# wesselb/stheno

Measured on AMD Instinct MI355X. Metric: GP logpdf+posterior evals/sec at N=16384 D=8 fp64, higher is better.
Workload: dtype f64; 1 GPU; EQ() kernel, N=16384 D=8 fp64, logpdf + condition, posterior mean/var at N*=2048; nan_scan=every step (the library's per-tensor memo is cleared at the start of each step), call_order=posterior-first, info_check=behind the call that factorised (the library's default), parallelism=replicas only (1 independent evals in flight, one process per GPU)

## Files before the change

### stheno_amd/csrc/gpk_common.hpp

```cpp
#pragma once
#include <hip/hip_runtime.h>
#include <stdint.h>
#include "../../include/gpk.h"

#ifdef GPK_DEV_KNOBS
#define GPK_KNOB(type, name, value) type name = (value)
#define GPK_KNOB_SET(stmt) stmt
#else
#define GPK_KNOB(type, name, value) constexpr type name = (value)
#define GPK_KNOB_SET(stmt) ((void)0)
#endif

#define GPK_WAVE 64
#define GPK_TILE 128
#define GPK_DB 128

#define GPK_ERR_ARG(i) (-(i))

typedef double f64x4 __attribute__((ext_vector_type(4)));
typedef float f32x4 __attribute__((ext_vector_type(4)));
typedef double f64x2 __attribute__((ext_vector_type(2)));

template <typename T>
struct Traits;

template <>
struct Traits<double> {
    typedef f64x4 acc_t;
    typedef f64x2 vec_t;
    static constexpr int VEC = 2;
    static constexpr int BK = 16;
    static __device__ __forceinline__ acc_t mfma(double a, double b, acc_t c) {
        return __builtin_amdgcn_mfma_f64_16x16x4f64(a, b, c, 0, 0, 0);
    }
    static __device__ __forceinline__ int crow(int lane, int i) { return (lane >> 4) + 4 * i; }
    static __host__ __device__ constexpr int rowq(int j) { return j & 3; }
    static __host__ __device__ constexpr int rowi(int j) { return j >> 2; }
};

template <>
struct Traits<float> {
    typedef f32x4 acc_t;
    typedef f32x4 vec_t;
    static constexpr int VEC = 4;
    static constexpr int BK = 32;
    static __device__ __forceinline__ acc_t mfma(float a, float b, acc_t c) {
        return __builtin_amdgcn_mfma_f32_16x16x4f32(a, b, c, 0, 0, 0);
    }
    static __device__ __forceinline__ int crow(int lane, int i) { return (lane >> 4) * 4 + i; }
    static __host__ __device__ constexpr int rowq(int j) { return j >> 2; }
    static __host__ __device__ constexpr int rowi(int j) { return j & 3; }
};

static inline int64_t gpk_cdiv(int64_t a, int64_t b) { return (a + b - 1) / b; }

#if defined(__HIPCC__)
__device__ __forceinline__ void gpk_barrier_stores_done() {
    asm volatile("s_waitcnt vmcnt(0)" ::: "memory");
    __syncthreads();
}
#endif

#define GPK_CHECK_LAUNCH()                                   \
    do {                                                     \
        hipError_t e__ = hipGetLastError();                  \
        if (e__ != hipSuccess) return GPK_ERR_LAUNCH;        \
    } while (0)


static inline bool gpk_valid_sb(int sb) { return sb >= 128 && sb <= 4096 && (sb & (sb - 1)) == 0; }

template <typename T>
int gpk_gemm_launch(bool a_kmaj, bool b_kmaj, int64_t M, int64_t N, int64_t K, T alpha,
                    const T* A, int64_t lda, int64_t sA, const T* B, int64_t ldb, int64_t sB,
                    T beta, T* C, int64_t ldc, int64_t sC, int64_t batch, int flags,
                    hipStream_t stream);

template <typename T>
int gpk_gemm_launch2(bool a_kmaj, bool b_kmaj, int64_t M, int64_t N, int64_t K, T alpha,
                     const T* A, int64_t lda, int64_t sA, int64_t sA2, const T* B, int64_t ldb,
                     int64_t sB, int64_t sB2, T beta, T* C, int64_t ldc, int64_t sC, int64_t sC2,
                     int64_t batch, int64_t batch2, int flags, hipStream_t stream,
                     const T* colscale = nullptr, T* colss = nullptr, int64_t ldss = 0);

#define GPK_PERSIST_CTRL_WORDS 64
int gpk_helper_stream(hipStream_t* aux, unsigned keys[8]);
int gpk_helper_side_stream(hipStream_t* side);
void gpk_helper_shutdown();
void gpk_potrf_shutdown();
template <typename T>
struct GpkSeg {
    int64_t M, N, K;
    const T* A; int64_t lda;
    const T* B; int64_t ldb;
    const T* Cin; int64_t ldcin;
    T* C; int64_t ldc;
    int lower_only;
    int signal;
    uint64_t colmask;
    int64_t grp;
};
#define GPK_PERSIST_MAX_SEG 4
struct GpkPersistSaved {
    alignas(16) char bytes[2048];
    int ts, edge, per_cu, valid;
    int signal_tiles;
};
template <typename T>
int gpk_gemm_persist_launch(const GpkSeg<T>* segs, int nseg, T alpha, unsigned* ctrl, int reserve,
                            hipStream_t stream, GpkPersistSaved* saved = nullptr, bool ctrl_zeroed = false);
template <typename T>
int gpk_gemm_persist_rejoin(const GpkPersistSaved* saved, hipStream_t helper_stream);

template <typename T>
int gpk_panel_step_launch(T* A, int64_t n, int64_t ld, int64_t c, const T* W, int64_t ke, unsigned* flags, hipStream_t stream);

template <typename T>
int gpk_potrf_launch(T* A, int64_t n, int64_t ld, int64_t batch, int64_t bstride, T* dinv,
                     int* info, int nbo, hipStream_t stream);

int64_t gpk_potrf_la_ws_elems_impl(int64_t n, int nb);
template <typename T>
int gpk_potrf_la_launch(T* A, int64_t n, int64_t ld, T* dinv128, T* dinv_big, int nb, T* ws, int* info,
                        hipStream_t stream, int sb = 0, int64_t rows = 0, int flags = 0);

template <typename T>
int gpk_potrf_rows_launch(T* A, int64_t n, int64_t rows, int64_t ld, T* dinv, int* info, hipStream_t stream);

void* gpk_prof_begin(int variant, double flops, hipStream_t stream);
void gpk_prof_end(void* slot, hipStream_t stream);

void gpk_tune_gemm(int key, int64_t value);
void gpk_tune_potrf(int key, int64_t value);
void gpk_tune_kmat(int key, int64_t value);
void gpk_tune_kdiff(int key, int64_t value);
void gpk_tune_solve(int key, int64_t value);
void gpk_set_diag_prof(long long* dev_buf);
void gpk_set_tile_prof(long long* dev_buf);
// ... 118 lines not shown
```

### stheno_amd/csrc/gpk_gemm.hip

```cpp
#include "gpk_common.hpp"
#include "gpk_gemm_tile.hpp"
#include <type_traits>
#include <cstring>
#include <mutex>
#include <vector>

namespace {

__device__ __forceinline__ void tri_decode(int s, int& I, int& J) {
    int i = (int)((sqrtf(8.f * (float)s + 1.f) - 1.f) * 0.5f);
    while ((i + 1) * (i + 2) / 2 <= s) ++i;
    while (i * (i + 1) / 2 > s) --i;
    I = i;
    J = s - i * (i + 1) / 2;
}

template <typename T>
__device__ __forceinline__ bool decode_tile(const GemmArgs<T>& p, int bid, int& ti, int& tj) {
    const bool tri = p.lower_only && p.tiles_m == p.tiles_n;
    if (tri) {
        tri_decode(bid, ti, tj);
        return ti < p.tiles_m;
    }
    if (p.tri_k_lo_b) {
// ... 232 lines not shown
    int variant;
    double flops;
    bool ended;
};
struct Prof {
    bool on = false;
    std::vector<ProfSlot> used, pool;
    ProfSlot* begin(int variant, double flops, hipStream_t stream) {
        ProfSlot s;
        if (!pool.empty()) {
            s = pool.back();
            pool.pop_back();
        } else {
            if (hipEventCreate(&s.a) != hipSuccess || hipEventCreate(&s.b) != hipSuccess) return nullptr;
        }
        s.variant = variant;
        s.flops = flops;
        s.ended = false;
        (void)hipEventRecord(s.a, stream);
        used.push_back(s);
        return &used.back();
    }
    void end(ProfSlot* s, hipStream_t stream) { (void)hipEventRecord(s->b, stream); s->ended = true; }
};
Prof g_prof;

GPK_KNOB(int64_t, g_small_tile_below, 512);
GPK_KNOB(int, g_trib, 1);
GPK_KNOB(int, g_xcd_batch, 1);
GPK_KNOB(int, g_trilo_pairs, 1);
GPK_KNOB(int, g_split_tail, 1);

}

namespace {
long long* g_tile_prof = nullptr;
int64_t g_tile_prof_only = -1;
int64_t g_tile_prof_count = 0;
GPK_KNOB(int64_t, g_persist_small_below, 512);
int g_cu_count[64] = {0};
int device_cus() {
    int dev = 0;
    if (hipGetDevice(&dev) != hipSuccess || dev < 0 || dev >= 64) return 256;
    if (g_cu_count[dev] == 0) {
        int n = 0;
        if (hipDeviceGetAttribute(&n, hipDeviceAttributeMultiprocessorCount, dev) != hipSuccess || n <= 0) n = 256;
        g_cu_count[dev] = n;
    }
    return g_cu_count[dev];
}
}

void gpk_set_tile_prof(long long* dev_buf) { g_tile_prof = dev_buf; }

void gpk_tune_gemm(int key, int64_t value) {
    if (key == 1) GPK_KNOB_SET(g_small_tile_below = value;);
    if (key == 8) GPK_KNOB_SET(g_persist_small_below = value;);
    if (key == 31) GPK_KNOB_SET(g_split_tail = (int)value;);
    if (key == 36) GPK_KNOB_SET(g_trib = (int)value;);
    if (key == 42) GPK_KNOB_SET(g_trilo_pairs = (int)value;);
    if (key == 45) GPK_KNOB_SET(g_xcd_batch = (int)value;);
    if (key == 20) { g_tile_prof_only = value; g_tile_prof_count = 0; }
}

void* gpk_prof_begin(int variant, double flops, hipStream_t stream) { return g_prof.on ? (void*)g_prof.begin(variant, flops, stream) : nullptr; }
void gpk_prof_end(void* slot, hipStream_t stream) {
    if (slot != nullptr) g_prof.end(static_cast<ProfSlot*>(slot), stream);
}

extern "C" int gpk_prof_start(void) {
    for (auto& s : g_prof.used) g_prof.pool.push_back(s);
    g_prof.used.clear();
    g_prof.on = true;
    return GPK_OK;
}

extern "C" int gpk_prof_stop(int variant, double* total_ms, int64_t* launches, double* useful_flops) {
    g_prof.on = false;
    double ms = 0, fl = 0;
    int64_t n = 0;
    for (auto& s : g_prof.used) {
        if (!s.ended) continue;
        if (hipEventSynchronize(s.b) != hipSuccess) return GPK_ERR_LAUNCH;
        if (variant >= 0 && s.variant != variant) continue;
        float t = 0;
        if (hipEventElapsedTime(&t, s.a, s.b) != hipSuccess) return GPK_ERR_LAUNCH;
        ms += t;
        fl += s.flops;
        ++n;
    }
    if (total_ms) *total_ms = ms;
    if (launches) *launches = n;
    if (useful_flops) *useful_flops = fl;
    return GPK_OK;
}

template <typename T>
int gpk_gemm_launch2(bool a_kmaj, bool b_kmaj, int64_t M, int64_t N, int64_t K, T alpha,
                     const T* A, int64_t lda, int64_t sA, int64_t sA2, const T* B, int64_t ldb,
                     int64_t sB, int64_t sB2, T beta, T* C, int64_t ldc, int64_t sC, int64_t sC2,
                     int64_t batch, int64_t batch2, int flags, hipStream_t stream, const T* colscale, T* colss, int64_t ldss) {
    const bool lower_only = (flags & 1) != 0;
    const bool fused_cols = colscale != nullptr || colss != nullptr;
    if (fused_cols && (batch != 1 || batch2 != 1 || lower_only || (const void*)A == (const void*)C || (const void*)B == (const void*)C))
        return GPK_ERR_ARG(17);
    if (M <= 0 || N <= 0 || batch <= 0 || batch2 <= 0) return GPK_OK;
// ... 519 lines not shown
```

### stheno_amd/csrc/gpk_gemm_tile.hpp

```cpp
#pragma once
#include "gpk_common.hpp"
#include <type_traits>

#ifndef GPK_GEMM_PIPE
#define GPK_GEMM_PIPE 2
#endif
#ifndef GPK_GEMM_PIPE64
#define GPK_GEMM_PIPE64 1
#endif
namespace {

constexpr int op_bytes(int ts) { return (ts + 16) * 128; }
constexpr int64_t GPK_PIPE_LD_MAX = (int64_t)1 << 21;
constexpr int64_t GPK_C_LD_MAX = (int64_t)1 << 25;

template <typename T>
struct GemmArgs {
    const T* A;
    const T* B;
    T* C;
    const T* Cin;
    int64_t lda, ldb, ldc, ldcin, sA, sB, sC;
    int64_t sA2, sB2, sC2;
    int M, N, K;
    T alpha, beta_over_alpha;
    int has_beta;
    int tiles_m, tiles_n;
    int lower_only;
    int vec_ok;
    int tri_k;
    int tri_k_lo;
    int tri_k_lo_b;
    int pair_cols;
    const T* colscale;
    T* colss;
    int64_t ldss;
    int xcd_batch;
    int xcd_tiles;
    unsigned long long colmask;
    int grp_tiles;
    int split_from;
};

__device__ __forceinline__ int gpk_claim_task(unsigned* ctr) { return (int)atomicAdd(ctr, 1u); }

template <typename T, int TS, bool KMAJ, bool EDGE, int NT = 256>
__device__ __forceinline__ void gload(typename Traits<T>::vec_t (&r)[TS * 8 / NT], const T* __restrict__ base,
                                      int64_t ld, int r0, int k0, int R, int K, int tid, bool fast) {
    typedef typename Traits<T>::vec_t vec_t;
    constexpr int VEC = Traits<T>::VEC;
    if (KMAJ) {
        const int c = tid & 7, rr0 = tid >> 3;
#pragma unroll
        for (int i = 0; i < TS * 8 / NT; ++i) {
            const int row = r0 + rr0 + (NT / 8) * i;
            const int k = k0 + c * VEC;
            const T* p = base + (int64_t)row * ld + k;
            if (!EDGE || fast) {
                r[i] = *reinterpret_cast<const vec_t*>(p);
            } else {
#pragma unroll
                for (int v = 0; v < VEC; ++v) r[i][v] = (row < R && k + v < K) ? p[v] : T(0);
            }
        }
    } else {
        constexpr int CPR = TS / VEC;
#pragma unroll
        for (int i = 0; i < TS * 8 / NT; ++i) {
            const int id = tid + NT * i;
            const int krow = id / CPR, cc = id % CPR;
            const int k = k0 + krow;
            const int row = r0 + cc * VEC;
            const T* p = base + (int64_t)k * ld + row;
            if (!EDGE || fast) {
                r[i] = *reinterpret_cast<const vec_t*>(p);
            } else {
#pragma unroll
                for (int v = 0; v < VEC; ++v) r[i][v] = (k < K && row + v < R) ? p[v] : T(0);
            }
        }
    }
}

template <typename T, int TS, bool KMAJ, int NT = 256>
__device__ __forceinline__ void sstore(char* lds, const typename Traits<T>::vec_t (&r)[TS * 8 / NT], int tid) {
    typedef typename Traits<T>::vec_t vec_t;
    constexpr int VEC = Traits<T>::VEC;
    if (KMAJ) {
        const int c = tid & 7, rr0 = tid >> 3;
#pragma unroll
        for (int i = 0; i < TS * 8 / NT; ++i) {
            const int rr = rr0 + (NT / 8) * i;
            const int off = rr * 128 + ((c ^ ((rr >> 1) & 7)) << 4);
            *reinterpret_cast<vec_t*>(lds + off) = r[i];
        }
    } else {
        constexpr int CPR = TS / VEC;
#pragma unroll
// ... 511 lines not shown
```

### stheno_amd/csrc/gpk_potrf.hip

```cpp
#include "gpk_common.hpp"
#include "gpk_gemm_tile.hpp"
#include "gpk_potrf_pipe.hpp"
#include <vector>

namespace {

constexpr int LDP = 130;

template <typename T>
struct DiagArgs {
    T* A;
    int64_t ld, bstride, off;
    int n;
    T* dinv;
    int64_t dinv_bstride;
    int* info;
    int info_base;
    long long* prof;
    int zero_next;
    T* rhs = nullptr;
    int64_t rhs_stride = 0;
};

#define PROF_MARK(i)                                                            \
// ... 449 lines not shown
    }
    int lane = lane_fixed;
    asm volatile("" : "+v"(lane));
    if (!vec_io) {
        for (int idx = tid; idx < GPK_DB * GPK_DB; idx += D3_THREADS) {
            const int r = idx >> 7, c = idx & 127;
            if (r < nv && c <= r) A[(int64_t)r * ld + c] = S[r * LDP + c];
        }
    }
    if (W == nullptr) {
        if (vec_io && wave == 4) store_l_columns<T>(S, A, ld, 7, lane);
        return;
    }
    if (prof) prof[10] = (long long)__builtin_readcyclecounter();

    inverse_last_rows<T>(S, rdiag, D16, W, wave, lane, lane & 15, lane >> 4);
    if (vec_io && wave == 7) store_l_columns<T>(S, A, ld, 7, lane);
    if (prof) prof[12] = (long long)__builtin_readcyclecounter();
    if (zero_next && tid < 256) {
        uint4* z = reinterpret_cast<uint4*>(W + (int64_t)GPK_DB * GPK_DB);
        z[tid] = make_uint4(0u, 0u, 0u, 0u);
    }
    if (prof) prof[13] = (long long)__builtin_readcyclecounter();
}


template <typename T, int WPE = 2>
__global__ __launch_bounds__(D3_THREADS, WPE) void potrf_diag3_kernel(DiagArgs<T> p) {
    __shared__ __attribute__((aligned(16))) T S[D3_LDS_ELEMS];
    const int64_t b = blockIdx.x;
    T* A = p.A + b * p.bstride + p.off * p.ld + p.off;
    const int rem = p.n - (int)p.off;
    T* W = p.dinv == nullptr ? nullptr : p.dinv + b * p.dinv_bstride + (p.off / GPK_DB) * (int64_t)(GPK_DB * GPK_DB);
    long long* prof = (p.prof != nullptr && blockIdx.x == 0 && threadIdx.x == 0) ? p.prof + (p.off / GPK_DB) * 32 : nullptr;
    diag3_block<T, true>(S, S + GPK_DB * LDP, A, p.ld, rem < GPK_DB ? rem : GPK_DB, W, p.info + b, (int)p.off + p.info_base, p.zero_next, prof);
    if (p.rhs != nullptr && W != nullptr) {
        gpk_barrier_stores_done();
        const int tid = threadIdx.x;
        const int nv = rem < GPK_DB ? rem : GPK_DB;
        T* yb = p.rhs + b * p.rhs_stride + p.off;
        if (tid < GPK_DB) S[tid] = tid < nv ? yb[tid] : T(0);
        __syncthreads();
        const int row = tid >> 2, q = tid & 3;
        const T* wr = W + (int64_t)row * GPK_DB + q * 32;
        T acc = T(0);
#pragma unroll 8
        for (int k = 0; k < 32; ++k) acc += wr[k] * S[q * 32 + k];
        acc += __shfl_xor(acc, 1, 64);
        acc += __shfl_xor(acc, 2, 64);
        if (q == 0 && row < nv) yb[row] = acc;
    }
}

constexpr unsigned PIPE_SPIN_LIMIT = 1u << 22;

template <typename T>
struct PipeArgs {
    T* A;
    int64_t ld;
    int m;
    int w;
    PipeShape sh;
    T* dinv;
    unsigned* ctrl;
    int* info;
    int info_off;
    int vec_ok;
    int ntasks, nseg;
    int segoff[GPK_PIPE_MAX_SEGS + 1];
    long long* prof;
    unsigned* wait_word;
    unsigned wait_value;
    GemmArgs<T> fill;
    int fill_tiles;
    int panel_wgs;
};

__device__ __forceinline__ bool pipe_poll(unsigned* w, bool mine, unsigned want, unsigned* abort_word) {
    unsigned it = 0;
    for (;;) {
        const bool ok = !mine || __hip_atomic_load(w, __ATOMIC_RELAXED, __HIP_MEMORY_SCOPE_AGENT) == want;
        if (__all(ok)) return true;
        __builtin_amdgcn_s_sleep(2);
        if ((++it & 255u) == 0) {
            if (__hip_atomic_load(abort_word, __ATOMIC_RELAXED, __HIP_MEMORY_SCOPE_AGENT) != 0u) return false;
            if (it > PIPE_SPIN_LIMIT) {
                __hip_atomic_store(abort_word, 1u, __ATOMIC_RELAXED, __HIP_MEMORY_SCOPE_AGENT);
                return false;
            }
        }
    }
}

__device__ __forceinline__ bool pipe_wait(unsigned* w0, unsigned* w1, unsigned* w2, unsigned* w3, unsigned v0, unsigned v1,
                                          unsigned v2, unsigned v3, int count, unsigned* abort_word, int* s_ctl) {
    const int tid = threadIdx.x;
    if (tid < 64) {
        unsigned* w = tid == 0 ? w0 : (tid == 1 ? w1 : (tid == 2 ? w2 : w3));
        const unsigned v = tid == 0 ? v0 : (tid == 1 ? v1 : (tid == 2 ? v2 : v3));
        const bool mine = tid < count;
        const bool ok = pipe_poll(mine ? w : w0, mine, v, abort_word);
        if (tid == 0) {
            s_ctl[1] = ok ? 1 : 0;
            __builtin_amdgcn_fence(__ATOMIC_ACQUIRE, "agent");
        }
    }
    __syncthreads();
    return s_ctl[1] != 0;
}

__device__ __forceinline__ void pipe_publish(unsigned* word, unsigned v, unsigned* counter = nullptr, unsigned full = 0u) {
    gpk_barrier_stores_done();
    if (threadIdx.x == 0) {
        __builtin_amdgcn_fence(__ATOMIC_RELEASE, "agent");
        asm volatile("s_waitcnt vmcnt(0)" ::: "memory");
        if (counter == nullptr) {
            __hip_atomic_store(word, v, __ATOMIC_RELAXED, __HIP_MEMORY_SCOPE_AGENT);
        } else {
            const unsigned before = __hip_atomic_fetch_add(counter, 1u, __ATOMIC_RELAXED, __HIP_MEMORY_SCOPE_AGENT);
            if (word != nullptr && before + 1u == full) __hip_atomic_store(word, v, __ATOMIC_RELAXED, __HIP_MEMORY_SCOPE_AGENT);
        }
    }
}

template <typename T>
__device__ __forceinline__ void pipe_chain(const PipeArgs<T>& p, T* __restrict__ S, int* s_ctl) {
    T* rdiag = S + GPK_DB * LDP;
    const int tid = threadIdx.x;
    const int npb = p.sh.npb, nd = p.sh.nd;
    unsigned* abort_word = p.ctrl + 1;
    unsigned* cnt = p.ctrl + GPK_PIPE_CTRL_HEAD + (int64_t)p.sh.R * npb;
    int64_t ld = p.ld;
    for (int j = 0; j < nd; ++j) {
        asm volatile("" : "+s"(ld));
        T* Ab = p.A + (int64_t)GPK_DB * j * ld + GPK_DB * j;
        const int rem = p.m - GPK_DB * j;
        T* W = p.dinv + (int64_t)j * (GPK_DB * GPK_DB);
        long long* prof = (p.prof != nullptr && tid == 0) ? p.prof + j * 32 : nullptr;
        if (prof) prof[14] = (long long)__builtin_readcyclecounter();
        if (j > 0) {
            unsigned* c = cnt + (int64_t)(2 * j) * npb + j;
            if (!pipe_wait(c, c, c, c, (unsigned)pipe_xupdates(pipe_fine_strips(p.sh, j - 1)), 0u, 0u, 0u, 1, abort_word, s_ctl)) break;
        } else if (p.wait_word != nullptr) {
            if (!pipe_wait(p.wait_word, p.wait_word, p.wait_word, p.wait_word, p.wait_value, 0u, 0u, 0u, 1, abort_word, s_ctl)) break;
        }
// ... 589 lines not shown
        bool done = false;
        if (owed > 0) {
            const T* P = A + k0 * ld + (k0 - owed);
            int st = gpk_gemm_launch<T>(true, true, rows - k0, k1 - k0, owed, T(-1), P, ld, bstride, P, ld, bstride, T(1), A + k0 * ld + k0, ld,
                                        bstride, batch, true, stream);
            if (st) return st;
            if (k1 < n && n - k0 > GPK_DB) {
                st = potrf_panel_pipe<T>(ctx, k0, nbo, &done, owed);
                if (st) return st;
            }
            if (!done && k1 < n) {
                const T* P2 = A + k1 * ld + (k0 - owed);
                st = gpk_gemm_launch<T>(true, true, rows - k1, n - k1, owed, T(-1), P2, ld, bstride, P2, ld, bstride, T(1), A + k1 * ld + k1, ld,
                                        bstride, batch, true, stream);
                if (st) return st;
            }
            owed = 0;
        }
        if (!done) {
            int pst = potrf_panel_any<T>(ctx, k0, nbo);
            if (pst) return pst;
        }
        if (k1 < n) {
            if (ride && n - k1 > GPK_DB) {
                owed = k1 - k0;
            } else {
                const T* P = A + k1 * ld + k0;
                int st = gpk_gemm_launch<T>(true, true, rows - k1, n - k1, k1 - k0, T(-1), P, ld, bstride, P, ld,
                                            bstride, T(1), A + k1 * ld + k1, ld, bstride, batch, true, stream);
                if (st) return st;
            }
        }
    }
    return GPK_OK;
}


#include <mutex>

namespace {

struct LaDevice {
    hipStream_t aux = nullptr;
    hipStream_t priv = nullptr;
    std::vector<hipEvent_t> events;
};
std::mutex g_la_mutex;
LaDevice g_la_dev[64];
GPK_KNOB(int64_t, g_la_min_rows, 2048);
GPK_KNOB(int64_t, g_la_tail_rows, 0);
GPK_KNOB(int, g_la_mode, 1);
GPK_KNOB(int64_t, g_la_fuse_diag_rows, 9216);
GPK_KNOB(int, g_la_fuse_diag_nb, 512);
GPK_KNOB(int, g_la_agg, 2);
GPK_KNOB(int64_t, g_la_agg_min_rows, 0);

LaDevice* la_device() {
    int dev = 0;
    if (hipGetDevice(&dev) != hipSuccess || dev < 0 || dev >= 64) return nullptr;
    LaDevice& d = g_la_dev[dev];
    if (d.aux == nullptr) {
        unsigned keys[8];
        if (gpk_helper_stream(&d.aux, keys) != GPK_OK) d.aux = nullptr;
    }
    return &d;
}

hipEvent_t la_event(LaDevice& d, size_t i) {
    while (d.events.size() <= i) {
        hipEvent_t e;
        if (hipEventCreateWithFlags(&e, hipEventDisableTiming) != hipSuccess) return nullptr;
        d.events.push_back(e);
    }
    return d.events[i];
}

template <typename T>
int la_chain(T* A, int64_t n, int64_t ld, T* dinv128, T* dinv_big, int nb, int sb, T* tmp, int* info, int64_t j,
             hipStream_t s, int max_wgs = 0, unsigned* wait_word = nullptr, unsigned wait_value = 0) {
    const int64_t k0 = j * nb;
    const int64_t w = (n - k0 < nb) ? n - k0 : nb;
    T* Ab = A + k0 * ld + k0;
    T* d128 = dinv128 + (k0 / GPK_DB) * (int64_t)(GPK_DB * GPK_DB);
    PanelCtx<T> sub{Ab, w, ld, 1, 0, d128, 0, info, s, (int)k0, max_wgs, wait_word, wait_value};
    int st = potrf_panel_any<T>(sub, 0, nb);
    if (st) return st;
    return gpk_trtri_merge_launch<T>(Ab, w, ld, 1, 0, d128, sb, dinv_big + (k0 / sb) * (int64_t)sb * sb, tmp, s);
}

}

void gpk_potrf_shutdown() {
    std::lock_guard<std::mutex> lock(g_la_mutex);
    int cur = 0;
    (void)hipGetDevice(&cur);
    for (int dev = 0; dev < 64; ++dev) {
        LaDevice& d = g_la_dev[dev];
        if (d.aux == nullptr && d.priv == nullptr && d.events.empty()) continue;
        (void)hipSetDevice(dev);
        if (d.priv != nullptr) {
            (void)hipStreamSynchronize(d.priv);
            (void)hipStreamDestroy(d.priv);
        }
        for (hipEvent_t e : d.events) (void)hipEventDestroy(e);
        d = LaDevice();
    }
    (void)hipSetDevice(cur);
}

void gpk_tune_potrf(int key, int64_t value) {
    if (key == 6) GPK_KNOB_SET(g_la_min_rows = value;);
    if (key == 7) GPK_KNOB_SET(g_la_mode = (int)value;);
    if (key == 9) GPK_KNOB_SET(g_la_tail_rows = value;);
    if (key == 32) GPK_KNOB_SET(g_fused_step = (int)value;);
    if (key == 37) GPK_KNOB_SET(g_pipe = (int)value;);
    if (key == 40) GPK_KNOB_SET(g_la_fuse_diag_rows = value;);
    if (key == 41) GPK_KNOB_SET(g_la_fuse_diag_nb = (int)value;);
    if (key == 47) GPK_KNOB_SET(g_la_agg = (int)value;);
    if (key == 48) GPK_KNOB_SET(g_la_agg_min_rows = value;);
    if (key == 52) GPK_KNOB_SET(g_plain_nbo = value;);
    if (key == 53) GPK_KNOB_SET(g_batch_mixed = (int)value;);
    if (key == 54) GPK_KNOB_SET(g_batch_mixed_min = value;);
    if (key == 55) GPK_KNOB_SET(g_batch_lag = (int)value;);
    if (key == 57) GPK_KNOB_SET(g_diag_two_per_cu = (int)value;);
    if (key == 38) GPK_KNOB_SET(g_pipe_fill = (int)value;);
    if (key == 39) GPK_KNOB_SET(g_pipe_panel_wgs = (int)value;);
}

#define GPK_LA_PAD 16
int64_t gpk_potrf_la_ws_elems_impl(int64_t n, int nb) {
    return (n > nb ? n : nb) * (int64_t)(nb + GPK_LA_PAD) + (int64_t)nb * nb / 4 + 16 + 128 + nb;
}

template <typename T>
static int potrf_la_body(LaDevice* dev, T* A, int64_t n, int64_t ld, T* dinv128, T* dinv_big, int nb, int sb, T* ws, int* info,
                         hipStream_t stream, int64_t rows, int flags);

template <typename T>
int gpk_potrf_la_launch(T* A, int64_t n, int64_t ld, T* dinv128, T* dinv_big, int nb, T* ws, int* info,
                        hipStream_t stream, int sb, int64_t rows, int flags) {
    if (n <= 0) return GPK_OK;
    if (rows < n) rows = n;
    if ((flags & GPK_ROWS_RHS) && rows < n + GPK_ROWS_RHS_STRIP) return GPK_ERR_ARG(2);
    if (rows > INT32_MAX) return GPK_ERR_ARG(2);
    if (rows > n && n % GPK_DB != 0) return GPK_ERR_ARG(2);
    if (rows > n && gpk_cdiv(n, nb) > 64) return GPK_ERR_ARG(2);
    if (ld < n) return GPK_ERR_ARG(3);
    if (nb < 256 || nb > 4096 || (nb & (nb - 1))) return GPK_ERR_ARG(6);
    if (sb <= 0) sb = nb;
    if (sb < 256 || sb > nb || (sb & (sb - 1))) return GPK_ERR_ARG(10);
    if (dinv128 == nullptr || dinv_big == nullptr || ws == nullptr || info == nullptr) return GPK_ERR_ARG(4);

    std::lock_guard<std::mutex> lock(g_la_mutex);
    LaDevice* dev = la_device();
    if (dev == nullptr) return GPK_ERR_LAUNCH;
    if (stream != nullptr) return potrf_la_body<T>(dev, A, n, ld, dinv128, dinv_big, nb, sb, ws, info, stream, rows, flags);

    if (dev->priv == nullptr && hipStreamCreateWithFlags(&dev->priv, hipStreamNonBlocking) != hipSuccess) {
        dev->priv = nullptr;
        return GPK_ERR_LAUNCH;
    }
    hipEvent_t e_in = la_event(*dev, 0), e_out = la_event(*dev, 1);
    if (e_in == nullptr || e_out == nullptr) return GPK_ERR_LAUNCH;
    if (hipEventRecord(e_in, nullptr) != hipSuccess || hipStreamWaitEvent(dev->priv, e_in, 0) != hipSuccess) return GPK_ERR_LAUNCH;
    const int st = potrf_la_body<T>(dev, A, n, ld, dinv128, dinv_big, nb, sb, ws, info, dev->priv, rows, flags);
    if (hipEventRecord(e_out, dev->priv) != hipSuccess || hipStreamWaitEvent(nullptr, e_out, 0) != hipSuccess) return st ? st : GPK_ERR_LAUNCH;
    return st;
}

template <typename T>
static int potrf_la_body(LaDevice* dev, T* A, int64_t n, int64_t ld, T* dinv128, T* dinv_big, int nb, int sb, T* ws, int* info,
                         hipStream_t stream, int64_t rows, int flags) {
    const bool rhs = (flags & GPK_ROWS_RHS) != 0;
    const int64_t Rall = rows;
    const int64_t R = rhs ? rows - GPK_ROWS_RHS_STRIP : rows;
    T* bvec = rhs ? A + R * ld : nullptr;
    unsigned* const ctrl_sets[2] = {reinterpret_cast<unsigned*>(ws), reinterpret_cast<unsigned*>(ws) + GPK_PERSIST_CTRL_WORDS};
    const int64_t ldt = nb + GPK_LA_PAD;
    T* Tp = ws + 128;
    T* tmp = Tp + (Rall > nb ? Rall : nb) * ldt;
    T* vtmp = tmp + (int64_t)nb * nb / 4 + 16;
    const int64_t nblk = gpk_cdiv(n, nb);
    const int64_t per = (int64_t)sb * sb;
    size_t ev = 2;

    auto finish_plain = [&](int64_t k) -> int {
        int s = potrf_plain<T>(A + k * ld + k, n - k, ld, 1, 0, dinv128 + (k / GPK_DB) * (int64_t)(GPK_DB * GPK_DB), info,
                               0, (int)k, stream, Rall - k);
        if (s) return s;
        if (flags & GPK_ROWS_NO_TAIL_INVERSES) return GPK_OK;
        return gpk_trtri_merge_launch<T>(A + k * ld + k, n - k, ld, 1, 0, dinv128 + (k / GPK_DB) * (int64_t)(GPK_DB * GPK_DB),
                                         sb, dinv_big + (k / sb) * per, Tp, stream);
    };
    int64_t tail_rows = g_la_tail_rows > 0 ? g_la_tail_rows : 6144;
    if (Rall > n && tail_rows < nb) tail_rows = nb;
    if (n <= tail_rows) return finish_plain(0);

    hipEvent_t e_side = nullptr;
    bool side_used = false;
    hipStream_t side = nullptr;
    if (rhs && g_la_mode == 1 && dev->aux != nullptr && gpk_helper_side_stream(&side) != GPK_OK) side = nullptr;
    auto rhs_panel = [&](int64_t j) -> int {
        if (!rhs) return GPK_OK;
        hipStream_t s = stream;
        if (side != nullptr) {
            hipEvent_t e = la_event(*dev, ev++);
            if (e == nullptr || hipEventRecord(e, stream) != hipSuccess || hipStreamWaitEvent(side, e, 0) != hipSuccess) return GPK_ERR_LAUNCH;
            side_used = true;
            s = side;
        }
        const int64_t k0 = j * nb;
        for (int64_t c = 0; c < nb; c += sb) {
            const int64_t r0 = k0 + c, r1 = r0 + sb;
            const int st1 = gpk_trsv_step_launch<T>(dinv_big + (r0 / sb) * per, sb, sb, A + r1 * ld + r0, ld, n - r1, bvec + r0, bvec + r1, vtmp, s);
            if (st1) return st1;
        }
        return GPK_OK;
    };
    auto rhs_join = [&]() -> int {
        if (!side_used) return GPK_OK;
        if (e_side == nullptr) e_side = la_event(*dev, ev++);
        if (e_side == nullptr || hipEventRecord(e_side, side) != hipSuccess || hipStreamWaitEvent(stream, e_side, 0) != hipSuccess) return GPK_ERR_LAUNCH;
        return GPK_OK;
    };
    auto steps = [&]() -> int {
        int st = la_chain<T>(A, n, ld, dinv128, dinv_big, nb, sb, tmp, info, 0, stream);
        if (st) return st;
        if (nblk > 1) {
            st = gpk_copy2d_launch<T>(A + (int64_t)nb * ld, ld, 0, Tp + (int64_t)nb * ldt, ldt, 0, R - nb, nb, 1, stream);
            if (st) return st;
        }
        const int agg = (g_la_agg > 1 && nblk <= 64) ? (int)g_la_agg : 1;
        std::vector<int> applied((size_t)nblk, 0);
        struct ColGroup { int from; uint64_t mask; };
        auto group_cols = [&](int64_t c_first, int64_t j, bool all, std::vector<ColGroup>& out) {
            out.clear();
            const bool wide = nblk - c_first > 64;
            for (int64_t c = c_first; c < nblk; ++c) {
                if (!all && (c - j) % agg != 0) continue;
                size_t g = 0;
                while (g < out.size() && out[g].from != applied[(size_t)c]) ++g;
                if (g == out.size()) out.push_back(ColGroup{applied[(size_t)c], 0});
                if (wide) out[g].mask = ~(uint64_t)0;
                else out[g].mask |= (uint64_t)1 << (c - c_first);
                applied[(size_t)c] = (int)(j + 1);
            }
        };
        auto col_segment = [&](const ColGroup& cg, int64_t c_first, int64_t k1) -> GpkSeg<T> {
            const int64_t kc = c_first * nb, ka = (int64_t)cg.from * nb;
            const T* P = A + kc * ld + ka;
            const uint64_t every = (nblk - c_first >= 64) ? ~(uint64_t)0 : (((uint64_t)1 << (nblk - c_first)) - 1);
            return GpkSeg<T>{R - kc, n - kc, k1 - ka, P, ld, P, ld, A + kc * ld + kc, ld, A + kc * ld + kc, ld, 1, 0,
                             (cg.mask == every && R == n) ? 0 : cg.mask, nb};
        };
        std::vector<ColGroup> groups;
        for (int64_t j = 0; j + 1 < nblk; ++j) {
            const int64_t k0 = j * nb, k1 = k0 + nb;
            const int64_t k2 = (k1 + nb < n) ? k1 + nb : n;
            unsigned* const ctrl_step = ctrl_sets[j & 1];
            unsigned* const ctrl = ctrl_sets[(j + 1) & 1];
            if (sb < nb) {
                for (int64_t i = 0; i * sb < nb && st == GPK_OK; ++i) {
                    const int64_t c = i * sb;
                    if (i > 0)
                        st = gpk_gemm_launch<T>(true, true, R - k1, sb, c, T(-1), A + k1 * ld + k0, ld, 0, A + (k0 + c) * ld + k0, ld, 0, T(1),
                                                Tp + k1 * ldt + c, ldt, 0, 1, 0, stream);
                    if (st == GPK_OK)
                        st = gpk_gemm_launch<T>(true, true, R - k1, sb, sb, T(1), Tp + k1 * ldt + c, ldt, 0, dinv_big + (k0 / sb + i) * per, sb, 0, T(0),
                                                A + k1 * ld + k0 + c, ld, 0, 1, 8, stream);
                }
            } else {
                st = gpk_gemm_launch<T>(true, true, R - k1, nb, nb, T(1), Tp + k1 * ldt, ldt, 0, dinv_big + j * per, nb, 0, T(0),
                                        A + k1 * ld + k0, ld, 0, 1, 8, stream);
            }
            if (st) return st;
            st = rhs_panel(j);
            if (st) return st;
            if (n - k1 <= tail_rows) {
                group_cols(j + 1, j, true, groups);
                for (size_t g0 = 0; g0 < groups.size(); g0 += GPK_PERSIST_MAX_SEG) {
                    GpkSeg<T> sg[GPK_PERSIST_MAX_SEG];
                    int ns = 0;
                    for (size_t g = g0; g < groups.size() && ns < GPK_PERSIST_MAX_SEG; ++g) sg[ns++] = col_segment(groups[g], j + 1, k1);
                    st = gpk_gemm_persist_launch<T>(sg, ns, T(-1), ctrl, 0, stream);
                    if (st) return st;
                }
                st = rhs_join();
                if (st) return st;
                return finish_plain(k1);
            }
            const int64_t ka1 = (int64_t)applied[(size_t)(j + 1)] * nb, kd1 = k1 - ka1;
            applied[(size_t)(j + 1)] = (int)(j + 1);
            const T* P1 = A + k1 * ld + ka1;
            const bool overlap = g_la_mode == 1 && dev->aux != nullptr && (n - k2) >= g_la_min_rows;
            const bool fuse_diag = overlap && nb <= g_la_fuse_diag_nb && g_la_fuse_diag_rows > 0 && (n - k2) >= g_la_fuse_diag_rows && g_pipe &&
                                   (k2 - k1) > GPK_DB;
            if (!fuse_diag) {
                st = gpk_gemm_launch<T>(true, true, k2 - k1, k2 - k1, kd1, T(-1), P1, ld, 0, P1, ld, 0, T(1),
                                        A + k1 * ld + k1, ld, 0, 1, 1, stream);
                if (st) return st;
            }
            if (k2 < n) group_cols(j + 2, j, agg == 1 || (n - k2) < g_la_agg_min_rows, groups);
            else groups.clear();
            {
                const size_t room = (size_t)(GPK_PERSIST_MAX_SEG - 1 - (fuse_diag ? 1 : 0));
                while (groups.size() > room) {
                    GpkSeg<T> sg = col_segment(groups.back(), j + 2, k1);
                    groups.pop_back();
                    st = gpk_gemm_persist_launch<T>(&sg, 1, T(-1), ctrl, 0, stream);
                    if (st) return st;
                }
            }
            hipEvent_t e_fork = nullptr, e_join = nullptr;
            if (overlap) {
                e_fork = la_event(*dev, ev++);
                e_join = la_event(*dev, ev++);
                if (e_fork == nullptr || e_join == nullptr) return GPK_ERR_LAUNCH;
                if (hipMemsetAsync(ctrl_step, 0, GPK_PERSIST_CTRL_WORDS * sizeof(unsigned), stream) != hipSuccess) return GPK_ERR_LAUNCH;
                if (hipEventRecord(e_fork, stream) != hipSuccess) return GPK_ERR_LAUNCH;
            } else {
                st = la_chain<T>(A, n, ld, dinv128, dinv_big, nb, sb, tmp, info, j + 1, stream);
                if (st) return st;
            }
            GpkPersistSaved saved;
            saved.valid = 0;
            auto forked = [&]() -> int {
                if (k2 < n) {
                    const T* P2 = A + k2 * ld + ka1;
                    GpkSeg<T> seg[GPK_PERSIST_MAX_SEG];
                    int ns = 0;
                    if (fuse_diag) seg[ns++] = GpkSeg<T>{k2 - k1, k2 - k1, kd1, P1, ld, P1, ld, A + k1 * ld + k1, ld, A + k1 * ld + k1, ld, 1, 1};
                    const GpkSeg<T> strip{R - k2, k2 - k1, kd1, P2, ld, P1, ld, A + k2 * ld + k1, ld, Tp + k2 * ldt, ldt, 0};
                    for (const ColGroup& cg : groups) seg[ns++] = col_segment(cg, j + 2, k1);
                    seg[ns++] = strip;
                    const int s2 = gpk_gemm_persist_launch<T>(seg, ns, T(-1), ctrl_step, overlap ? 1 : 0, stream, &saved, overlap);
                    if (s2) return s2;
                }
                if (overlap) {
                    if (hipStreamWaitEvent(dev->aux, e_fork, 0) != hipSuccess) return GPK_ERR_LAUNCH;
                    const int s2 = fuse_diag ? la_chain<T>(A, n, ld, dinv128, dinv_big, nb, sb, tmp, info, j + 1, dev->aux, 8, ctrl_step + 2, (unsigned)saved.signal_tiles)
                                             : la_chain<T>(A, n, ld, dinv128, dinv_big, nb, sb, tmp, info, j + 1, dev->aux, 8);
                    if (s2) return s2;
                    if (saved.valid)
                        return gpk_gemm_persist_rejoin<T>(&saved, dev->aux);
                }
                return GPK_OK;
            };
            st = forked();
            if (overlap) {
                const bool joined = hipEventRecord(e_join, dev->aux) == hipSuccess && hipStreamWaitEvent(stream, e_join, 0) == hipSuccess;
                if (!joined && st == GPK_OK) st = GPK_ERR_LAUNCH;
            }
            if (st) return st;
        }
        return GPK_OK;
    };
    const int st_all = steps();
    const int st_join = rhs_join();
    return st_all ? st_all : st_join;
}

template int gpk_potrf_la_launch<double>(double*, int64_t, int64_t, double*, double*, int, double*, int*, hipStream_t, int, int64_t, int);
template int gpk_potrf_la_launch<float>(float*, int64_t, int64_t, float*, float*, int, float*, int*, hipStream_t, int, int64_t, int);

template <typename T>
int gpk_potrf_launch(T* A, int64_t n, int64_t ld, int64_t batch, int64_t bstride, T* dinv,
                     int* info, int nbo, hipStream_t stream) {
    return potrf_plain<T>(A, n, ld, batch, bstride, dinv, info, nbo, 0, stream);
}

template <typename T>
int gpk_potrf_rhs_launch(T* A, int64_t n, int64_t ld, int64_t batch, int64_t bstride, T* dinv, int* info, int nbo, T* B, int64_t sB, T* tmp,
                         hipStream_t stream) {
    if (B == nullptr || tmp == nullptr || dinv == nullptr) return GPK_ERR_ARG(9);
    if (batch > 1 && sB < n) return GPK_ERR_ARG(10);
    RhsRide<T> ride{B, sB, tmp, false};
    int st = potrf_plain<T>(A, n, ld, batch, bstride, dinv, info, nbo, 0, stream, 0, &ride);
    if (st) return st;
    if (!ride.done) st = gpk_trsv_launch<T>(A, n, ld, bstride, dinv, GPK_DB, B, 1, 1, sB, tmp, batch, stream);
    return st;
}
template int gpk_potrf_rhs_launch<double>(double*, int64_t, int64_t, int64_t, int64_t, double*, int*, int, double*, int64_t, double*, hipStream_t);
template int gpk_potrf_rhs_launch<float>(float*, int64_t, int64_t, int64_t, int64_t, float*, int*, int, float*, int64_t, float*, hipStream_t);

template <typename T>
int gpk_potrf_rows_launch(T* A, int64_t n, int64_t rows, int64_t ld, T* dinv, int* info, hipStream_t stream) {
    return potrf_plain<T>(A, n, ld, 1, 0, dinv, info, 0, 0, stream, rows);
}
// ... 8 lines not shown
```

Before: 28.72 evals/s.

## Add solve+diagonal-SYRK rider kernel and run last-step RHS panel in-line

Adds a fused kernel for the blocked Cholesky: the last panel-solve GEMM and the next diagonal-block SYRK run in one launch. Rider workgroups poll per-row counters published by the solve tiles, so the diagonal update starts as soon as its input rows are done. This is meant to remove one launch and the serial gap before the SYRK, at the cost of spin-waiting and ordering risk; it sits behind a knob that defaults to off. Separately, and on by default, the last step's RHS panel now runs in-line on the main stream after the tail updates instead of forking to the side stream, avoiding event fork/join overhead. `pipe_poll` moves into a shared header.

```diff
diff --git a/stheno_amd/csrc/gpk_common.hpp b/stheno_amd/csrc/gpk_common.hpp
--- a/stheno_amd/csrc/gpk_common.hpp
+++ b/stheno_amd/csrc/gpk_common.hpp
@@ -16,6 +16,7 @@
 #define GPK_DB 128
 
 #define GPK_ERR_ARG(i) (-(i))
+#define GPK_PERSIST_CTRL_WORDS 64
 
 typedef double f64x4 __attribute__((ext_vector_type(4)));
 typedef float f32x4 __attribute__((ext_vector_type(4)));
@@ -77,13 +78,17 @@
                     hipStream_t stream);
 
 template <typename T>
+int gpk_gemm_solve_rider_launch(int64_t M, int64_t N, int64_t K, const T* A, int64_t lda, const T* B, int64_t ldb, T* C, int64_t ldc,
+                                int64_t nd, int64_t kd, const T* P, int64_t ldp, T* D, int64_t ldd, unsigned* ctrl, unsigned* zero,
+                                int* info, hipStream_t stream, bool* taken);
+
+template <typename T>
 int gpk_gemm_launch2(bool a_kmaj, bool b_kmaj, int64_t M, int64_t N, int64_t K, T alpha,
                      const T* A, int64_t lda, int64_t sA, int64_t sA2, const T* B, int64_t ldb,
                      int64_t sB, int64_t sB2, T beta, T* C, int64_t ldc, int64_t sC, int64_t sC2,
                      int64_t batch, int64_t batch2, int flags, hipStream_t stream,
                      const T* colscale = nullptr, T* colss = nullptr, int64_t ldss = 0);
 
-#define GPK_PERSIST_CTRL_WORDS 64
 int gpk_helper_stream(hipStream_t* aux, unsigned keys[8]);
 int gpk_helper_side_stream(hipStream_t* side);
 void gpk_helper_shutdown();
diff --git a/stheno_amd/csrc/gpk_gemm.hip b/stheno_amd/csrc/gpk_gemm.hip
--- a/stheno_amd/csrc/gpk_gemm.hip
+++ b/stheno_amd/csrc/gpk_gemm.hip
@@ -308,6 +308,7 @@
 }
 
 void gpk_set_tile_prof(long long* dev_buf) { g_tile_prof = dev_buf; }
+int64_t gpk_gemm_small_tile_below() { return g_small_tile_below; }
 
 void gpk_tune_gemm(int key, int64_t value) {
     if (key == 1) GPK_KNOB_SET(g_small_tile_below = value;);
diff --git a/stheno_amd/csrc/gpk_gemm_rider.hip b/stheno_amd/csrc/gpk_gemm_rider.hip
--- /dev/null
+++ b/stheno_amd/csrc/gpk_gemm_rider.hip
@@ -0,0 +1,141 @@
+#include "gpk_common.hpp"
+#include "gpk_gemm_tile.hpp"
+
+int64_t gpk_gemm_small_tile_below();
+
+namespace {
+
+__device__ __forceinline__ void rider_tri_decode(int s, int& I, int& J) {
+    int i = (int)((sqrtf(8.f * (float)s + 1.f) - 1.f) * 0.5f);
+    while ((i + 1) * (i + 2) / 2 <= s) ++i;
+    while (i * (i + 1) / 2 > s) --i;
+    I = i;
+    J = s - i * (i + 1) / 2;
+}
+
+template <typename T>
+struct SolveRiderArgs {
+    GemmArgs<T> solve, rider;
+    unsigned* rowcnt;
+    unsigned* abort_word;
+    unsigned* zero;
+    int* info;
+    int nd;
+    int n_rider, rider_at;
+};
+
+template <typename T>
+__global__ __launch_bounds__(256, 2) void solve_rider_kernel(SolveRiderArgs<T> p) {
+    __shared__ __attribute__((aligned(16))) char smem[2 * 2 * op_bytes(128)];
+    const int tid = threadIdx.x;
+    int bid = (int)blockIdx.x;
+    if (bid == 0 && p.zero != nullptr && tid < GPK_PERSIST_CTRL_WORDS) p.zero[tid] = 0u;
+    if (bid >= p.rider_at && bid < p.rider_at + p.n_rider) {
+        int r2, c2;
+        rider_tri_decode(bid - p.rider_at, r2, c2);
+        typedef __attribute__((address_space(3))) volatile int lds_word_t;
+        lds_word_t& s_ok = *(lds_word_t*)(uint32_t)(uintptr_t)smem;
+        if (tid < 64) {
+            const bool mine = tid < 2;
+            const bool ok = pipe_poll(p.rowcnt + ((tid == 1 ? c2 : r2) >> 1), mine, (unsigned)p.solve.tiles_n, p.abort_word);
+            if (tid == 0) {
+                s_ok = ok ? 1 : 0;
+                __builtin_amdgcn_fence(__ATOMIC_ACQUIRE, "agent");
+                asm volatile("s_waitcnt vmcnt(0)" ::: "memory");
+            }
+        }
+        __syncthreads();
+        const bool ok = s_ok != 0;
+        __syncthreads();
+        if (!ok) {
+            if (tid == 0) atomicExch(p.info, -1);
+            return;
+        }
+        gemm_tile<T, 64, true, true, false, 1, 4, false, GPK_GEMM_PIPE>(p.rider, r2, c2, 0, 0, smem);
+        return;
+    }
+    if (bid >= p.rider_at) bid -= p.n_rider;
+    const GemmArgs<T>& g = p.solve;
+    const int head = p.nd * g.tiles_n;
+    int ti, tj;
+    if (bid < head) {
+        const int c = bid / p.nd;
+        tj = g.tiles_n - 1 - c;
+        ti = bid - c * p.nd;
+    } else {
+        const int rest = g.tiles_m - p.nd, s = bid - head;
+        const int c = s / rest;
+        tj = g.tiles_n - 1 - c;
+        ti = p.nd + (s - c * rest);
+        if (tj < 0) return;
+    }
+    gemm_tile<T, 128, true, true, false, 1, 4, false, GPK_GEMM_PIPE>(g, ti, tj, 0, 0, smem);
+    if (ti < p.nd) {
+        gpk_barrier_stores_done();
+        if (tid == 0) {
+            __builtin_amdgcn_fence(__ATOMIC_RELEASE, "agent");
+            asm volatile("s_waitcnt vmcnt(0)" ::: "memory");
+            __hip_atomic_fetch_add(&p.rowcnt[ti], 1u, __ATOMIC_RELAXED, __HIP_MEMORY_SCOPE_AGENT);
+        }
+    }
+}
+
+}
+
+template <typename T>
+int gpk_gemm_solve_rider_launch(int64_t M, int64_t N, int64_t K, const T* A, int64_t lda, const T* B, int64_t ldb, T* C, int64_t ldc,
+                                int64_t nd, int64_t kd, const T* P, int64_t ldp, T* D, int64_t ldd, unsigned* ctrl, unsigned* zero,
+                                int* info, hipStream_t stream, bool* taken) {
+    *taken = false;
+    if (ctrl == nullptr || info == nullptr) return GPK_OK;
+    constexpr int VEC = Traits<T>::VEC;
+    constexpr int BK = Traits<T>::BK;
+    if (M <= 0 || N <= 0 || nd <= 0 || M > INT32_MAX || kd > INT32_MAX) return GPK_OK;
+    if (M % 128 || N % 128 || K % BK || K < BK || nd % 128 || nd > M || kd % BK || kd < BK) return GPK_OK;
+    const int64_t tm = M / 128, tn = N / 128, ndt = nd / 128;
+    if (tm * tn < gpk_gemm_small_tile_below() || 16 + ndt > GPK_PERSIST_CTRL_WORDS) return GPK_OK;
+    const bool aligned = ((uintptr_t)A % 16 == 0) && ((uintptr_t)B % 16 == 0) && ((uintptr_t)P % 16 == 0) && (lda % VEC == 0) &&
+                         (ldb % VEC == 0) && (ldp % VEC == 0);
+    if (!aligned || lda >= GPK_PIPE_LD_MAX || ldb >= GPK_PIPE_LD_MAX || ldp >= GPK_PIPE_LD_MAX || ldc >= GPK_C_LD_MAX || ldd >= GPK_C_LD_MAX)
+        return GPK_OK;
+    const int64_t t64 = 2 * ndt, n_rider = t64 * (t64 + 1) / 2;
+    if (tm * tn + n_rider > INT32_MAX / 2) return GPK_OK;
+
+    SolveRiderArgs<T> p;
+    auto fill = [](GemmArgs<T>& g, const T* a, int64_t la, const T* b, int64_t lb, T* c, int64_t lc, int64_t m, int64_t n, int64_t k, int ts) {
+        g.A = a; g.B = b; g.C = c; g.Cin = c;
+        g.lda = la; g.ldb = lb; g.ldc = lc; g.ldcin = lc;
+        g.sA = g.sB = g.sC = g.sA2 = g.sB2 = g.sC2 = 0;
+        g.M = (int)m; g.N = (int)n; g.K = (int)k;
+        g.tiles_m = (int)(m / ts); g.tiles_n = (int)(n / ts);
+        g.vec_ok = 1;
+        g.lower_only = g.tri_k = g.tri_k_lo = g.tri_k_lo_b = g.pair_cols = 0;
+        g.colscale = nullptr; g.colss = nullptr; g.ldss = 0;
+        g.xcd_batch = g.xcd_tiles = 0; g.colmask = 0; g.grp_tiles = 0;
+        g.split_from = INT32_MAX;
+    };
+    fill(p.solve, A, lda, B, ldb, C, ldc, M, N, K, 128);
+    p.solve.alpha = T(1); p.solve.has_beta = 0; p.solve.beta_over_alpha = T(0);
+    p.solve.tri_k_lo_b = 1;
+    fill(p.rider, P, ldp, P, ldp, D, ldd, nd, nd, kd, 64);
+    p.rider.alpha = T(-1); p.rider.has_beta = 1; p.rider.beta_over_alpha = T(1) / T(-1);
+    p.rider.lower_only = 1;
+    p.abort_word = ctrl + 8;
+    p.rowcnt = ctrl + 16;
+    p.zero = zero;
+    p.info = info;
+    p.nd = (int)ndt;
+    p.n_rider = (int)n_rider;
+    const int64_t n_solve = tm * tn;
+    p.rider_at = (int)n_solve;
+    void* slot = gpk_prof_begin((sizeof(T) == 8 ? 8 : 0) + 4 + 2, (double)M * (double)N * (double)K + (double)nd * (double)nd * (double)kd, stream);
+    hipLaunchKernelGGL((solve_rider_kernel<T>), dim3((unsigned)(n_solve + n_rider)), dim3(256), 0, stream, p);
+    gpk_prof_end(slot, stream);
+    GPK_CHECK_LAUNCH();
+    *taken = true;
+    return GPK_OK;
+}
+template int gpk_gemm_solve_rider_launch<double>(int64_t, int64_t, int64_t, const double*, int64_t, const double*, int64_t, double*, int64_t, int64_t,
+                                                 int64_t, const double*, int64_t, double*, int64_t, unsigned*, unsigned*, int*, hipStream_t, bool*);
+template int gpk_gemm_solve_rider_launch<float>(int64_t, int64_t, int64_t, const float*, int64_t, const float*, int64_t, float*, int64_t, int64_t,
+                                                int64_t, const float*, int64_t, float*, int64_t, unsigned*, unsigned*, int*, hipStream_t, bool*);
diff --git a/stheno_amd/csrc/gpk_gemm_tile.hpp b/stheno_amd/csrc/gpk_gemm_tile.hpp
--- a/stheno_amd/csrc/gpk_gemm_tile.hpp
+++ b/stheno_amd/csrc/gpk_gemm_tile.hpp
@@ -44,6 +44,23 @@
 
 __device__ __forceinline__ int gpk_claim_task(unsigned* ctr) { return (int)atomicAdd(ctr, 1u); }
 
+constexpr unsigned PIPE_SPIN_LIMIT = 1u << 22;
+__device__ __forceinline__ bool pipe_poll(unsigned* w, bool mine, unsigned want, unsigned* abort_word) {
+    unsigned it = 0;
+    for (;;) {
+        const bool ok = !mine || __hip_atomic_load(w, __ATOMIC_RELAXED, __HIP_MEMORY_SCOPE_AGENT) == want;
+        if (__all(ok)) return true;
+        __builtin_amdgcn_s_sleep(2);
+        if ((++it & 255u) == 0) {
+            if (__hip_atomic_load(abort_word, __ATOMIC_RELAXED, __HIP_MEMORY_SCOPE_AGENT) != 0u) return false;
+            if (it > PIPE_SPIN_LIMIT) {
+                __hip_atomic_store(abort_word, 1u, __ATOMIC_RELAXED, __HIP_MEMORY_SCOPE_AGENT);
+                return false;
+            }
+        }
+    }
+}
+
 template <typename T, int TS, bool KMAJ, bool EDGE, int NT = 256>
 __device__ __forceinline__ void gload(typename Traits<T>::vec_t (&r)[TS * 8 / NT], const T* __restrict__ base,
                                       int64_t ld, int r0, int k0, int R, int K, int tid, bool fast) {
diff --git a/stheno_amd/csrc/gpk_potrf.hip b/stheno_amd/csrc/gpk_potrf.hip
--- a/stheno_amd/csrc/gpk_potrf.hip
+++ b/stheno_amd/csrc/gpk_potrf.hip
@@ -525,7 +525,6 @@
     }
 }
 
-constexpr unsigned PIPE_SPIN_LIMIT = 1u << 22;
 
 template <typename T>
 struct PipeArgs {
@@ -548,22 +547,6 @@
     int fill_tiles;
     int panel_wgs;
 };
-
-__device__ __forceinline__ bool pipe_poll(unsigned* w, bool mine, unsigned want, unsigned* abort_word) {
-    unsigned it = 0;
-    for (;;) {
-        const bool ok = !mine || __hip_atomic_load(w, __ATOMIC_RELAXED, __HIP_MEMORY_SCOPE_AGENT) == want;
-        if (__all(ok)) return true;
-        __builtin_amdgcn_s_sleep(2);
-        if ((++it & 255u) == 0) {
-            if (__hip_atomic_load(abort_word, __ATOMIC_RELAXED, __HIP_MEMORY_SCOPE_AGENT) != 0u) return false;
-            if (it > PIPE_SPIN_LIMIT) {
-                __hip_atomic_store(abort_word, 1u, __ATOMIC_RELAXED, __HIP_MEMORY_SCOPE_AGENT);
-                return false;
-            }
-        }
-    }
-}
 
 __device__ __forceinline__ bool pipe_wait(unsigned* w0, unsigned* w1, unsigned* w2, unsigned* w3, unsigned v0, unsigned v1,
                                           unsigned v2, unsigned v3, int count, unsigned* abort_word, int* s_ctl) {
@@ -1259,6 +1242,8 @@
 GPK_KNOB(int, g_la_mode, 1);
 GPK_KNOB(int64_t, g_la_fuse_diag_rows, 9216);
 GPK_KNOB(int, g_la_fuse_diag_nb, 512);
+GPK_KNOB(int, g_la_solve_rider, 0);
+GPK_KNOB(int, g_la_rhs_last_inline, 1);
 GPK_KNOB(int, g_la_agg, 2);
 GPK_KNOB(int64_t, g_la_agg_min_rows, 0);
 
@@ -1323,6 +1308,8 @@
     if (key == 37) GPK_KNOB_SET(g_pipe = (int)value;);
     if (key == 40) GPK_KNOB_SET(g_la_fuse_diag_rows = value;);
     if (key == 41) GPK_KNOB_SET(g_la_fuse_diag_nb = (int)value;);
+    if (key == 61) GPK_KNOB_SET(g_la_solve_rider = (int)value;);
+    if (key == 63) GPK_KNOB_SET(g_la_rhs_last_inline = (int)value;);
     if (key == 47) GPK_KNOB_SET(g_la_agg = (int)value;);
     if (key == 48) GPK_KNOB_SET(g_la_agg_min_rows = value;);
     if (key == 52) GPK_KNOB_SET(g_plain_nbo = value;);
@@ -1407,10 +1394,10 @@
     bool side_used = false;
     hipStream_t side = nullptr;
     if (rhs && g_la_mode == 1 && dev->aux != nullptr && gpk_helper_side_stream(&side) != GPK_OK) side = nullptr;
-    auto rhs_panel = [&](int64_t j) -> int {
+    auto rhs_panel = [&](int64_t j, bool in_line = false) -> int {
         if (!rhs) return GPK_OK;
         hipStream_t s = stream;
-        if (side != nullptr) {
+        if (side != nullptr && !in_line) {
             hipEvent_t e = la_event(*dev, ev++);
             if (e == nullptr || hipEventRecord(e, stream) != hipSuccess || hipStreamWaitEvent(side, e, 0) != hipSuccess) return GPK_ERR_LAUNCH;
             side_used = true;
@@ -1431,6 +1418,7 @@
         return GPK_OK;
     };
     auto steps = [&]() -> int {
+        if (g_la_solve_rider && hipMemsetAsync(ctrl_sets[0], 0, 2 * GPK_PERSIST_CTRL_WORDS * sizeof(unsigned), stream) != hipSuccess) return GPK_ERR_LAUNCH;
         int st = la_chain<T>(A, n, ld, dinv128, dinv_big, nb, sb, tmp, info, 0, stream);
         if (st) return st;
         if (nblk > 1) {
@@ -1466,24 +1454,41 @@
             const int64_t k2 = (k1 + nb < n) ? k1 + nb : n;
             unsigned* const ctrl_step = ctrl_sets[j & 1];
             unsigned* const ctrl = ctrl_sets[(j + 1) & 1];
+            const bool last_step = n - k1 <= tail_rows;
+            const int64_t ka1 = (int64_t)applied[(size_t)(j + 1)] * nb, kd1 = k1 - ka1;
+            const T* P1 = A + k1 * ld + ka1;
+            const bool overlap = !last_step && g_la_mode == 1 && dev->aux != nullptr && (n - k2) >= g_la_min_rows;
+            const bool fuse_diag = overlap && nb <= g_la_fuse_diag_nb && g_la_fuse_diag_rows > 0 && (n - k2) >= g_la_fuse_diag_rows && g_pipe &&
+                                   (k2 - k1) > GPK_DB;
+            bool rode = false;
+            auto solve_last = [&](int64_t N_, int64_t K_, const T* Ap, const T* Bp, int64_t ldb_, T* Cp) -> int {
+                if (g_la_solve_rider && !last_step && !fuse_diag) {
+                    const int s1 = gpk_gemm_solve_rider_launch<T>(R - k1, N_, K_, Ap, ldt, Bp, ldb_, Cp, ld, k2 - k1, kd1, P1, ld, A + k1 * ld + k1, ld,
+                                                                  ctrl, ctrl_step, info, stream, &rode);
+                    if (s1 || rode) return s1;
+                }
+                return gpk_gemm_launch<T>(true, true, R - k1, N_, K_, T(1), Ap, ldt, 0, Bp, ldb_, 0, T(0), Cp, ld, 0, 1, 8, stream);
+            };
             if (sb < nb) {
                 for (int64_t i = 0; i * sb < nb && st == GPK_OK; ++i) {
                     const int64_t c = i * sb;
                     if (i > 0)
                         st = gpk_gemm_launch<T>(true, true, R - k1, sb, c, T(-1), A + k1 * ld + k0, ld, 0, A + (k0 + c) * ld + k0, ld, 0, T(1),
                                                 Tp + k1 * ldt + c, ldt, 0, 1, 0, stream);
-                    if (st == GPK_OK)
+                    if (st == GPK_OK && c + sb < nb)
                         st = gpk_gemm_launch<T>(true, true, R - k1, sb, sb, T(1), Tp + k1 * ldt + c, ldt, 0, dinv_big + (k0 / sb + i) * per, sb, 0, T(0),
                                                 A + k1 * ld + k0 + c, ld, 0, 1, 8, stream);
+                    else if (st == GPK_OK)
+                        st = solve_last(sb, sb, Tp + k1 * ldt + c, dinv_big + (k0 / sb + i) * per, sb, A + k1 * ld + k0 + c);
                 }
             } else {
-                st = gpk_gemm_launch<T>(true, true, R - k1, nb, nb, T(1), Tp + k1 * ldt, ldt, 0, dinv_big + j * per, nb, 0, T(0),
-                                        A + k1 * ld + k0, ld, 0, 1, 8, stream);
+                st = solve_last(nb, nb, Tp + k1 * ldt, dinv_big + j * per, nb, A + k1 * ld + k0);
             }
             if (st) return st;
-            st = rhs_panel(j);
+            const bool rhs_in_line = last_step && g_la_rhs_last_inline;
+            if (!rhs_in_line) st = rhs_panel(j);
             if (st) return st;
-            if (n - k1 <= tail_rows) {
+            if (last_step) {
                 group_cols(j + 1, j, true, groups);
                 for (size_t g0 = 0; g0 < groups.size(); g0 += GPK_PERSIST_MAX_SEG) {
                     GpkSeg<T> sg[GPK_PERSIST_MAX_SEG];
@@ -1492,17 +1497,14 @@
                     st = gpk_gemm_persist_launch<T>(sg, ns, T(-1), ctrl, 0, stream);
                     if (st) return st;
                 }
+                if (rhs_in_line) st = rhs_panel(j, true);
+                if (st) return st;
                 st = rhs_join();
                 if (st) return st;
                 return finish_plain(k1);
             }
-            const int64_t ka1 = (int64_t)applied[(size_t)(j + 1)] * nb, kd1 = k1 - ka1;
             applied[(size_t)(j + 1)] = (int)(j + 1);
-            const T* P1 = A + k1 * ld + ka1;
-            const bool overlap = g_la_mode == 1 && dev->aux != nullptr && (n - k2) >= g_la_min_rows;
-            const bool fuse_diag = overlap && nb <= g_la_fuse_diag_nb && g_la_fuse_diag_rows > 0 && (n - k2) >= g_la_fuse_diag_rows && g_pipe &&
-                                   (k2 - k1) > GPK_DB;
-            if (!fuse_diag) {
+            if (!fuse_diag && !rode) {
                 st = gpk_gemm_launch<T>(true, true, k2 - k1, k2 - k1, kd1, T(-1), P1, ld, 0, P1, ld, 0, T(1),
                                         A + k1 * ld + k1, ld, 0, 1, 1, stream);
                 if (st) return st;
@@ -1523,7 +1525,7 @@
                 e_fork = la_event(*dev, ev++);
                 e_join = la_event(*dev, ev++);
                 if (e_fork == nullptr || e_join == nullptr) return GPK_ERR_LAUNCH;
-                if (hipMemsetAsync(ctrl_step, 0, GPK_PERSIST_CTRL_WORDS * sizeof(unsigned), stream) != hipSuccess) return GPK_ERR_LAUNCH;
+                if (!rode && hipMemsetAsync(ctrl_step, 0, GPK_PERSIST_CTRL_WORDS * sizeof(unsigned), stream) != hipSuccess) return GPK_ERR_LAUNCH;
                 if (hipEventRecord(e_fork, stream) != hipSuccess) return GPK_ERR_LAUNCH;
             } else {
                 st = la_chain<T>(A, n, ld, dinv128, dinv_big, nb, sb, tmp, info, j + 1, stream);
@@ -1540,7 +1542,7 @@
                     const GpkSeg<T> strip{R - k2, k2 - k1, kd1, P2, ld, P1, ld, A + k2 * ld + k1, ld, Tp + k2 * ldt, ldt, 0};
                     for (const ColGroup& cg : groups) seg[ns++] = col_segment(cg, j + 2, k1);
                     seg[ns++] = strip;
-                    const int s2 = gpk_gemm_persist_launch<T>(seg, ns, T(-1), ctrl_step, overlap ? 1 : 0, stream, &saved, overlap);
+                    const int s2 = gpk_gemm_persist_launch<T>(seg, ns, T(-1), ctrl_step, overlap ? 1 : 0, stream, &saved, overlap || rode);
                     if (s2) return s2;
                 }
                 if (overlap) {
```

Result: no change. 28.85 evals/s (median of 6 runs) (+0.4%).
